# OxfordML/GPz

Measured on AMD Instinct MI355X. Metric: objective+gradient evals/sec, higher is better.
Workload: dtype f64

## Files before the change

gpz_amd/csrc/gpz_ctx.h:

```cpp
#pragma once
#include <hip/hip_runtime.h>
#include <math.h>
#include <stdarg.h>
#include <stdio.h>
#include <stdlib.h>
#include <string.h>
#include <algorithm>
#include <atomic>
#include <mutex>
#include <string>
#include <type_traits>
#include <vector>
#include "../../include/gpz_hip.h"
#include "gpz_dev.h"
#include "gpz_kernels.h"
#include <map>

#define HIPCHK(x)                                                                                   \
    do {                                                                                            \
        hipError_t e_ = (x);                                                                        \
        if (e_ != hipSuccess) return gpz_fail(GPZ_ERR_HIP, "%s:%d %s: %s", __FILE__, __LINE__, #x, hipGetErrorString(e_)); \
    } while (0)

inline int method_id_of(const char *m) {
// ... 129 lines not shown
    }
    hipEvent_t get() {
        if (pool_used == pool.size()) {
            hipEvent_t e;
            (void)hipEventCreate(&e);
            pool.push_back(e);
        }
        return pool[pool_used++];
    }
};

struct gpz_ctx {
    gpz_desc desc;
    gpz_options opt = gpz_options_load();
    int mid = 0, kind = 0, d = 0, de = 0, m = 0, mp = 0, mq = 0, k = 1, hetero = 0, g_dim = 0;
    long p = 0;
    int device = 0;
    hipStream_t st = nullptr;
    Arena ar;
    RowSet tr, va;
    double *theta_d = nullptr;
    GpzParams pr{};
    double *Phi = nullptr, *T = nullptr, *dL = nullptr;
    double *lnbeta = nullptr, *wbeta = nullptr, *phiw = nullptr;
    double *lnbeta_v = nullptr, *phiw_v = nullptr;
    double *slab = nullptr;
    size_t slab_count = 0;
    int nsplit = 1, rows_per_split = 16;
    int nsplit_d = 1, rows_per_split_d = 16;
    int nsplit_l = 1, rows_per_split_l = 16;
    double *comm1 = nullptr;
    size_t comm1_count = 0;
    double *comm2 = nullptr;
    size_t comm2_count = 0;
    int nm = 0;
    double *A = nullptr, *Lm = nullptr, *Wm = nullptr, *Tmp = nullptr, *Sinv = nullptr, *Bext = nullptr;
    float *Bext32 = nullptr;
    char *oz_A = nullptr, *oz_B = nullptr;
    double *oz_cs = nullptr;
    double *w = nullptr, *dwda = nullptr, *dgi = nullptr, *logdet = nullptr;
    int *info = nullptr;
    double *colslab = nullptr, *scal_slab = nullptr;
    int nwg_rows = 1;
    double *mom_slab = nullptr;
    int nchunk = 1, rows_per_chunk = 1;
    int tile_rows = 0, ntiles = 1, tile_nchunk = 1, tile_rpc = 1;
    double *tile_rstats = nullptr;
    double *partial = nullptr, *rstats = nullptr, *dGfull = nullptr, *spart = nullptr;
    double *nupart = nullptr, *rowscal = nullptr, *frec = nullptr;
    bool syrk_small = false;
    bool small_tail_dp = false;
    bool small_tail = false;
    int st_nwg = 0, st_nf = 0;
    double *st_slab = nullptr;
    bool fused = true;
    double *phipart = nullptr;
    int phipart_groups = 0;
    long phipart_rows = 0;
    int nslots = 0;
    double *out_d = nullptr;
    double *out_h = nullptr, *theta_h = nullptr;
    gpz_allreduce_fn ar_fn = nullptr;
    void *ar_user = nullptr;
    void *priv = nullptr;
    void (*priv_free)(void *) = nullptr;
    int timing = 0;
    bool time_rest = false;
    struct GraphSeg {
        hipGraphExec_t exec = nullptr;
        int stage = -1;
        bool count_call = false;
        double *hook_buf = nullptr;
        size_t hook_count = 0;
    };
    struct GraphSet { std::vector<GraphSeg> segs; int state = 0; };
    GraphSet gset[2];
    GraphSet *cap = nullptr;
    int cap_stage = -1;
    bool cap_stage_first = false, cap_failed = false;
    hipStream_t graph_st = nullptr;
    bool capturing = false;
    StageTimer tm;
    bool phi_valid = false;
    bool has_psi = false, has_missing = false;
    int pinv_mode = 0;
    double *g_dev_out = nullptr;
    double pinv_last[4] = {0, 0, 0, 0};
    bool gen = false;
    bool psi_fast = false;
    bool psi_miss = false;
    bool psi32 = false;
    int psi_kind_in = 0;
    bool need_psi3 = true;
    bool psi32_agreed = false;
    int ngroups = 0, nrec = 0;
    std::vector<std::vector<unsigned char>> pats;
    bool pats_fixed = false;
    unsigned char *pat_d = nullptr;
    double *prep_ws = nullptr;
    double *Sig = nullptr, *iSig = nullptr, *lnS = nullptr, *Phi_v = nullptr, *gen_slab = nullptr, *psi32_raw = nullptr;
    double *gc_minv = nullptr;
    double *gcq_A = nullptr, *gcq_B = nullptr;
    double *RcP = nullptr, *gen_tslab = nullptr, *gen_frec = nullptr, *fin_part = nullptr;
    double *gen_ws = nullptr;
    int gen_tnch = 1;
    int *mom_chunktab = nullptr, *mom_segtab = nullptr;
// ... 66 lines not shown
```

gpz_amd/csrc/gpz_ctx.hip:

```cpp
#include "gpz_ctx.h"

namespace gpzi {
static int upload_rowset(gpz_ctx *c, RowSet &rs, int64_t n_tot, const double *X, const double *Y, const double *omega,
                         const uint8_t *mask, bool need_xr, const double *Psi = nullptr) {
    const int d = c->d, de = c->de, k = c->k;
    std::vector<int64_t> idx;
    idx.reserve((size_t)n_tot);
    for (int64_t i = 0; i < n_tot; ++i)
        if (!mask || mask[i]) idx.push_back(i);
    if (c->gen) {
        std::vector<int> hg0(idx.size());
        for (size_t r = 0; r < idx.size(); ++r) {
            std::vector<unsigned char> pt(d);
            for (int c_ = 0; c_ < d; ++c_) { const double xv = X[(size_t)c_ * n_tot + idx[r]]; pt[c_] = (xv != xv) ? 0 : 1; }
            int g = -1;
            for (size_t q = 0; q < c->pats.size(); ++q)
                if (c->pats[q] == pt) { g = (int)q; break; }
            if (g < 0) {
                if (c->pats_fixed) return gpz_fail(GPZ_ERR_ARG, "row %lld has a NaN pattern that is not in the given pattern table", (long long)idx[r]);
                c->pats.push_back(pt);
                g = (int)c->pats.size() - 1;
            }
            hg0[r] = g;
        }
// ... 464 lines not shown
        int target = rows_at(1024) >= 16384 ? 1024 : rows_at(512) >= 4096 ? 512 : 256;
        if (c->opt.syrk_wgs > 0) target = c->opt.syrk_wgs;
        const int noff = npairs - nt, max_ns = np_k / 64 > 0 ? (int)(np_k / 64) : 1;
        int s1 = 1, s2 = 1;
        double best = 1e300;
        for (int a = 1; a <= max_ns && a <= target && noff * a + nt <= (target > npairs ? target : npairs); ++a) {
            int b = noff ? (target - noff * a) / nt : a;
            if (b > max_ns) b = max_ns;
            if (b > a) b = a;
            if (b < 1) b = 1;
            const double cost = 1.0 / a > 0.6 / b ? 1.0 / a : 0.6 / b;
            if (cost < best) { best = cost; s1 = a; s2 = b; }
        }
        if (c->opt.syrk_s1 > 0) s1 = c->opt.syrk_s1;
        if (c->opt.syrk_s2 > 0) s2 = c->opt.syrk_s2;
        c->rows_per_split = rup((int)((np_k + s1 - 1) / s1), 16);
        c->nsplit = (int)((np_k + c->rows_per_split - 1) / c->rows_per_split);
        c->rows_per_split_d = rup((int)((np_k + s2 - 1) / s2), 16);
        c->nsplit_d = (int)((np_k + c->rows_per_split_d - 1) / c->rows_per_split_d);
        size_t need = (size_t)(c->nsplit > c->nsplit_d ? c->nsplit : c->nsplit_d) * mp * mp;
        c->syrk_small = syrk_small_fits(mp) && !c->psi32 && !c->opt.syrk_small_off;
        if (c->syrk_small) {
            const size_t ns = syrk_small_slab_count((int)np_k, mp);
            if (ns > need) need = ns;
        }
        size_t need_l = (size_t)c->nsplit_l * c->mq * c->mq;
        c->slab_count = need > need_l ? need : need_l;
        if ((rc = c->ar.alloc(&c->slab, c->slab_count))) return bail(rc);
    }
    {
        size_t prow = npt < 1024 * 1024 ? npt : 0;
        if (c->va.n_pad && (size_t)c->va.n_pad < 1024 * 1024 && (size_t)c->va.n_pad > prow) prow = (size_t)c->va.n_pad;
        if (prow) {
            c->phipart_groups = 16;
            c->phipart_rows = (long)prow;
            if ((rc = c->ar.alloc(&c->phipart, (size_t)c->phipart_groups * 2 * k * prow))) return bail(rc);
        }
    }
    c->comm1_count = k * mp * mp + gpz_ns(c->k);
    if ((rc = c->ar.alloc(&c->comm1, c->comm1_count))) return bail(rc);
    c->comm2_count = m * c->nm + k * 2 * mp + k * 4 + gpz_ns(c->k);
    if ((rc = c->ar.alloc(&c->comm2, c->comm2_count))) return bail(rc);
    c->nwg_rows = c->tr.n < 2048 ? (c->tr.n > 0 ? c->tr.n : 1) : 2048;
    if (!c->fused) {
        if ((rc = c->ar.alloc(&c->colslab, (size_t)c->nwg_rows * 2 * mp))) return bail(rc);
        if ((rc = c->ar.alloc(&c->scal_slab, (size_t)c->nwg_rows * 4))) return bail(rc);
    } else {
        c->nslots = gpz_gemm_wave_cols() * ((c->mp + 127) / 128);
        if ((rc = c->ar.alloc(&c->nupart, (size_t)c->nslots * npt))) return bail(rc);
        if ((rc = c->ar.alloc(&c->rowscal, (size_t)4 * np))) return bail(rc);
        if ((rc = c->ar.alloc(&c->frec, (size_t)m * (c->nm + 2)))) return bail(rc);
    }
    {
        const int ncg = (c->m + 255) / 256;
        const int nc_env = c->opt.mom_nc;
        int nc = nc_env > 0 ? nc_env / ncg : (768 / ncg > 512 ? 768 / ncg : (2048 / ncg < 512 ? 2048 / ncg : 512));
        if (nc_env <= 0 && c->kind == GPZ_KIND_COV) {
            long rounds = ((long)c->tr.n * ncg + 1024 * 1000 - 1) / (1024 * 1000);
            if (rounds < 1) rounds = 1;
            if (rounds > 4) rounds = 4;
            nc = (int)(512 * rounds / ncg);
            if (nc < 1) nc = 1;
        }
        if (nc_env <= 0 && c->kind == GPZ_KIND_DIAG && c->m < 256) nc = nc * 256 / ((c->m + 63) / 64 * 64);
        const int max_nc = c->tr.n / 32 > 0 ? c->tr.n / 32 : 1;
        if (nc > max_nc) nc = max_nc;
        if (nc < 1) nc = 1;
        if (c->gen) nc = 1;
        c->rows_per_chunk = (c->tr.n + nc - 1) / nc;
        if (c->rows_per_chunk < 1) c->rows_per_chunk = 1;
        c->nchunk = c->tr.n > 0 ? (c->tr.n + c->rows_per_chunk - 1) / c->rows_per_chunk : 1;
        if (c->tile_rows) {
            int nct = nc;
            if (nct > c->tile_rows / 32) nct = c->tile_rows / 32 > 0 ? c->tile_rows / 32 : 1;
            c->tile_rpc = (c->tile_rows + nct - 1) / nct;
            c->tile_nchunk = (c->tile_rows + c->tile_rpc - 1) / c->tile_rpc;
            c->nchunk = c->ntiles * c->tile_nchunk;
        }
        if ((rc = c->ar.alloc(&c->mom_slab, (size_t)c->nchunk * m * (c->nm + 2)))) return bail(rc);
    }
    if ((rc = c->ar.alloc(&c->partial, (size_t)GPZ_ROWSCAL_MAX_NWG * gpz_ns(c->k)))) return bail(rc);
    static_assert(GPZ_ROWSCAL_MAX_NWG >= GPZ_SMALL_NWG, "partial record buffer");
    if ((rc = c->ar.alloc(&c->rstats, (size_t)gpz_ns(c->k)))) return bail(rc);
    if ((rc = c->ar.alloc(&c->spart, (size_t)(c->k > 8 ? c->k : 8)))) return bail(rc);
    if ((rc = c->ar.alloc(&c->dGfull, c->kind == GPZ_KIND_COV ? m * c->d * c->d : m * c->d))) return bail(rc);
    if ((rc = c->ar.alloc(&c->out_d, (size_t)c->p + 10))) return bail(rc);
    if (hipHostMalloc((void **)&c->out_h, ((size_t)c->p + 10) * sizeof(double)) != hipSuccess ||
        hipHostMalloc((void **)&c->theta_h, (size_t)c->p * sizeof(double)) != hipSuccess)
        return bail(gpz_fail(GPZ_ERR_ALLOC, "hipHostMalloc failed"));
    *out = c;
    return GPZ_OK;
}
namespace gpzi {

}
extern "C" void gpz_ctx_destroy(gpz_ctx *c) {
    if (!c) return;
    (void)hipSetDevice(c->device);
    (void)hipStreamSynchronize(c->st);
    if (c->priv && c->priv_free) c->priv_free(c->priv);
    c->ar.release();
    if (c->out_h) (void)hipHostFree(c->out_h);
    if (c->theta_h) (void)hipHostFree(c->theta_h);
    for (auto &gs : c->gset)
        for (auto &s : gs.segs)
            if (s.exec) (void)hipGraphExecDestroy(s.exec);
    if (c->graph_st) (void)hipStreamDestroy(c->graph_st);
    for (hipEvent_t e : c->tm.pool) (void)hipEventDestroy(e);
    delete c;
}
namespace gpzi {

}
bool gpz_ctx_allreduce_is(const gpz_ctx *c, int (*fn)(void *, void *, size_t, void *), void **user) {
    if (user) *user = c->ar_user;
    return c->ar_fn == fn;
}
int gpz_ctx_device(const gpz_ctx *c) { return c->device; }
void gpz_ctx_attach_private(gpz_ctx *c, void *priv, void (*free_fn)(void *)) {
    if (c->priv && c->priv_free) c->priv_free(c->priv);
    c->priv = priv;
    c->priv_free = free_fn;
}
namespace gpzi {

}
extern "C" int gpz_ctx_set_allreduce(gpz_ctx *c, gpz_allreduce_fn fn, void *user) {
    if (!c) return gpz_fail(GPZ_ERR_ARG, "null context");
    c->ar_fn = fn;
    c->ar_user = user;
    return GPZ_OK;
}
// ... 37 lines not shown
    c->timing = enable < 0 ? 0 : enable > 2 ? 2 : enable;
    c->time_rest = enable >= 3;
    return GPZ_OK;
}
namespace gpzi {
}
extern "C" int gpz_ctx_reset_timings(gpz_ctx *c) {
    if (!c) return gpz_fail(GPZ_ERR_ARG, "null context");
    for (auto &v : c->tm.ms) v = 0.0;
    for (auto &v : c->tm.calls) v = 0;
    return GPZ_OK;
}
namespace gpzi {
}
extern "C" int gpz_ctx_timings(gpz_ctx *c, const char **names, double *ms, int64_t *calls, int cap) {
    if (!c) return gpz_fail(GPZ_ERR_ARG, "null context");
    const int n = (int)c->tm.names.size();
    for (int i = 0; i < n && i < cap; ++i) {
        if (names) names[i] = c->tm.names[i];
        if (ms) ms[i] = c->tm.ms[i];
        if (calls) calls[i] = c->tm.calls[i];
    }
    return n;
}
namespace gpzi {

}
extern "C" int gpz_ctx_route(const gpz_ctx *c, char *buf, int cap) {
    if (!c || !buf || cap <= 0) return gpz_fail(GPZ_ERR_ARG, "gpz_ctx_route: null argument");
    const bool f32req = c->desc.dtype == GPZ_F32;
    const char *phi, *why = "";
    if (!c->gen) phi = c->d > 20 ? "tuned diagonal / covariance kernels, runtime-d form (k_wide)" : "tuned kernels (k_phi, k_rows)";
    else if (!c->has_psi) phi = "covariance kinds with missing dimensions: tuned kernels per NaN pattern";
    else if (c->psi32) phi = (c->tr.psi_diag && psi32m_available(c->d))
                                 ? "fp32 pair kernels: k_psi32_phi + k_psi32m_moments (4x4 MFMA tiles)" : "fp32 pair kernels (k_psi32)";
    else if (c->psi_fast) phi = c->d <= 10 ? "fp64 pair kernels in registers (k_psi)"
                                : cpsi4_available(c->d) ? "fp64 pair kernels on 4x4 f64 MFMA tiles (k_cpsi4)" : "fp64 pair kernels on MFMA tiles (k_cpsi4w / k_cpsi)";
    else phi = "fp64 pair kernels, workspace form (k_gen)";
    if (f32req && !c->psi32)
        why = !c->gen || !c->has_psi ? " [dtype f32 requested: no input noise on a covariance kind, nothing runs in fp32]"
              : c->d > 20            ? " [dtype f32 requested: d > 20 has no fp32 pair kernel, fp64 route]"
                                     : " [dtype f32 requested: rows with missing dimensions, fp64 route]";
    const int gstate = c->gset[c->timing == 2 ? 1 : 0].state;
    const size_t nseg = c->gset[c->timing == 2 ? 1 : 0].segs.size();
    char gsb[96];
    if (gstate == 2 && nseg > 1) snprintf(gsb, sizeof gsb, "replayed (%zu segments%s)", nseg, c->desc.world > 1 ? ", all-reduce between them" : "");
    else snprintf(gsb, sizeof gsb, "%s", gstate == 2 ? "replayed" : gstate == -1 ? "disabled (recording failed)" : c->opt.no_graph ? "disabled (GPZ_NO_GRAPH)"
                                         : c->timing == 1 ? "off (stage timing on)" : "eager (not recorded yet)");
    const char *gs = gsb;
    const bool f32mm = c->psi32 && !c->opt.f32_contractions_off;
    char rows[96];
    if (c->tile_rows) snprintf(rows, sizeof rows, "; rows: streamed, %d tiles of %d (PHI built twice per evaluation)", c->ntiles, c->tile_rows);
    else rows[0] = 0;
    return snprintf(buf, (size_t)cap, "pair/PHI kernels: %s%s; contractions: %s MFMA%s%s; evaluation graph: %s%s", phi, why,
                    f32mm ? "fp32-operand (fp64 master sums)" : "fp64",
                    c->syrk_small ? ", PHI' W PHI with the whole triangle in one workgroup (k_syrk_small)" : "",
                    c->small_tail ? ", T-GEMM + row scalars + moments in one kernel (k_small_tail: T stays in registers)" :
                    c->small_tail_dp ? ", T-GEMM + row scalars + dPHI in one kernel (k_small_tail; moment sums with input noise by k_moments_diag)" : "", gs, rows);
}
namespace gpzi {

}
```

gpz_amd/csrc/gpz_eval.hip:

```cpp
#include "gpz_ctx.h"

namespace gpzi {
static GenRows gen_rows(const RowSet &rs) {
    GenRows r{};
    r.Xr = rs.Xr; r.gid = rs.gid; r.Psi3 = rs.Psi3; r.rows_by_group = rs.rows_by_group; r.n = rs.n; r.n_pad = rs.n_pad;
    return r;
}

static void psi32_chunks(const gpz_ctx *c, int *nch, int *rpc) {
    int r = (c->tr.n + c->gen_nchunk - 1) / c->gen_nchunk;
    r = rup(r > 0 ? r : 1, 64);
    *rpc = r;
    *nch = c->tr.n > 0 ? (c->tr.n + r - 1) / r : 1;
}

static int allreduce(gpz_ctx *c, double *buf, size_t count) {
    if (c->desc.world <= 1) return 0;
    if (!c->ar_fn) return gpz_fail(GPZ_ERR_COMM, "world=%d but no all-reduce hook set (gpz_ctx_set_allreduce)", c->desc.world);
    if (c->capturing) {
        if (graph_cut(c)) return gpz_fail(GPZ_ERR_HIP, "evaluation graph: cut at an exchange point failed");
        c->cap->segs.back().hook_buf = buf;
        c->cap->segs.back().hook_count = count;
        return 0;
    }
// ... 261 lines not shown
        if (c->pinv_mode == 0) launch_cond_flag(c->st, S, c->mp, c->pr.alpha + (size_t)o * m, c->Sinv, mq, m, c->Tmp, c->info);
    }
}

static int stage_b_pinv(gpz_ctx *c, int o) {
    const int mq = c->mq, m = c->m;
    const double *S = c->comm1 + (size_t)o * c->mp * c->mp;
    Stage s(c, "pinv_svd");
    double *sbuf = c->Tmp, *out3 = c->Tmp + mq + 8;
    unsigned long long *word = (unsigned long long *)(c->Tmp + mq);
    const int sweeps = run_jacobi_pinv(c->st, S, c->mp, c->pr.alpha + (size_t)o * m, m, c->A, c->Wm, mq, sbuf, word, c->Sinv,
                                       mq, c->logdet + o, out3);
    if (sweeps < 0) return gpz_fail(GPZ_ERR_HIP, "pseudo-inverse (Jacobi SVD) failed: %s", hipGetErrorString(hipGetLastError()));
    double h3[3] = {0, 0, 0};
    HIPCHK(hipMemcpyAsync(h3, out3, sizeof h3, hipMemcpyDeviceToHost, c->st));
    HIPCHK(hipStreamSynchronize(c->st));
    c->pinv_last[0] = 1.0;
    c->pinv_last[1] = (o == 0) ? h3[1] : fmin(c->pinv_last[1], h3[1]);
    c->pinv_last[2] = h3[2];
    c->pinv_last[3] = (double)sweeps;
    launch_post_inverse(c->st, c->Sinv, mq, S, c->mp, c->pr.alpha + (size_t)o * m, m, c->mp, o, c->Bext,
                        c->w + (size_t)o * m, c->dwda + (size_t)o * m, c->dgi + (size_t)o * m, c->info, c->logdet);
    return 0;
}

int eval_tail(gpz_ctx *c, bool pinv) {
    const size_t mp = c->mp, m = c->m, k = c->k;
    double *mom = c->comm2;
    double *cols = mom + m * c->nm;
    double *scal = cols + k * 2 * mp;
    double *vsums = scal + k * 4;
    const bool fused = c->fused;
    for (int o = 0; o < c->k; ++o) {
        if (pinv) { if (int e = stage_b_pinv(c, o)) return e; }
        else stage_b(c, o);
        if (c->tile_rows) {
            const size_t oo = (size_t)o * c->tr.n_pad;
            for (int t = 0; t < c->ntiles; ++t) {
                const RowTile rt = row_tile(c, t);
                const long r0 = rt.r0;
                { Stage s(c, "phi_build"); if (int e = phi_tile(c, rt)) return e; }
                {
                    Stage s(c, "tgemm");
                    launch_tgemm(c->st, c->Phi, c->mp, c->Bext, c->mp, c->T, rt.rows_pad, c->mp, c->nupart, c->phiw + oo + r0, c->m, c->m + o,
                                 c->psi32 && !c->opt.f32_contractions_off);
                }
                {
                    Stage s(c, "row_scalars");
                    launch_row_scalars(c->st, c->nupart, c->nslots, c->phiw + oo + r0, c->tr.Y + oo + r0, c->tr.om ? c->tr.om + r0 : nullptr,
                                       c->lnbeta + oo + r0, c->wbeta + oo + r0, rt.rows_pad, rt.rows, c->rowscal + 4 * r0, c->partial, (long)o * c->tr.om_ld);
                    launch_slab_sum(c->st, c->partial, row_scalars_nwg(rt.rows), GPZ_NS, c->tile_rstats + (size_t)t * GPZ_NS);
                }
                Stage s(c, "moments");
                FusedMomentArgs a{};
                a.Phi = c->Phi; a.T = c->T; a.ld = c->mp; a.Xr = c->tr.Xr + r0 * c->de; a.rowscal = c->rowscal + 4 * r0; a.n = rt.rows;
                a.m = c->m; a.d = c->de; a.kind = c->kind; a.P = c->pr.P; a.w = c->w + (size_t)o * m;
                a.v = c->hetero ? c->pr.v + (size_t)o * m : nullptr;
                a.rows_per_chunk = c->tile_rpc; a.nchunk = (rt.rows + c->tile_rpc - 1) / c->tile_rpc;
                a.slab = c->mom_slab + (size_t)t * c->tile_nchunk * m * (c->nm + 2); a.nm = c->nm;
                a.Psir = c->tr.Psir ? c->tr.Psir + r0 * c->de : nullptr; a.Mr = c->tr.Mr ? c->tr.Mr + r0 * c->de : nullptr; a.G2 = c->pr.G2;
                if (a.nchunk > 0 && launch_moments_fused(c->st, a))
                    return gpz_fail(GPZ_ERR_UNSUPPORTED, "moment kernel not instantiated for d=%d", c->de);
            }
            Stage s(c, "moments");
            launch_slab_sum(c->st, c->tile_rstats, c->ntiles, GPZ_NS, c->rstats);
            HIPCHK(hipMemcpyAsync(scal + (size_t)o * 4, c->rstats, 4 * sizeof(double), hipMemcpyDeviceToDevice, c->st));
            const RowTile last = row_tile(c, c->ntiles - 1);
            const int nch = (c->ntiles - 1) * c->tile_nchunk + (last.rows + c->tile_rpc - 1) / c->tile_rpc;
            launch_slab_sum(c->st, c->mom_slab, nch, m * (c->nm + 2), c->frec);
            launch_split_fused(c->st, c->frec, c->m, c->nm, c->mp, mom, cols + (size_t)o * 2 * mp, o > 0 ? 1 : 0);
            continue;
        }
        if (c->small_tail_dp) {
            {
                Stage s(c, "tail_small");
                SmallTailArgs a{};
                a.Phi = c->Phi; a.ld = c->mp; a.B = c->Bext; a.ldb = c->mp;
                a.n = c->tr.n; a.n_pad = c->tr.n_pad; a.m = c->m; a.mp = c->mp; a.d = c->de; a.kind = c->kind; a.mcol = c->m;
                a.Xs = c->tr.Xs; a.xs_ld = c->tr.xs_ld; a.missing = 0;
                a.y = c->tr.Y; a.omega = c->tr.om; a.omega1 = c->tr.om; a.lnbeta = c->lnbeta; a.wbeta = c->wbeta;
                a.w = c->w; a.v = c->hetero ? c->pr.v : c->w; a.vscale = c->hetero ? 1.0 : 0.0;
                a.phiw = c->phiw; a.slab = c->st_slab; a.partial = c->partial; a.nf = 0; a.stagger = c->opt.small_stagger;
                a.dphi = c->T; a.ldd = c->mp;
                launch_small_tail(c->st, a, c->st_nwg);
                launch_small_finish(c->st, c->st_slab, c->partial, c->st_nwg, c->m, c->de, c->kind, 0, 0, c->pr.P, c->tr.xmu, c->nm, c->mp, mom,
                                    cols, scal, 0, 1);
            }
            Stage s(c, "moments");
            MomentArgs ma{};
            ma.dPhi = c->T; ma.ld = c->mp; ma.Xr = c->tr.Xr; ma.n = c->tr.n; ma.n_pad = c->tr.n_pad; ma.m = c->m; ma.d = c->de;
            ma.kind = c->kind; ma.P = c->pr.P; ma.nchunk = c->nchunk; ma.rows_per_chunk = c->rows_per_chunk; ma.slab = c->mom_slab;
            ma.nm = c->nm; ma.Psir = c->tr.Psir; ma.Mr = c->tr.Mr; ma.G2 = c->pr.G2;
            if (launch_moments(c->st, ma)) return gpz_fail(GPZ_ERR_UNSUPPORTED, "moment kernel not instantiated for d=%d", c->de);
            launch_slab_sum(c->st, c->mom_slab, c->nchunk, m * c->nm, mom);
            continue;
        }
        if (c->small_tail) {
            Stage s(c, "tail_small");
            const size_t oo = (size_t)o * c->tr.n_pad;
            SmallTailArgs a{};
            a.Phi = c->Phi; a.ld = c->mp; a.B = c->Bext; a.ldb = c->mp;
            a.n = c->tr.n; a.n_pad = c->tr.n_pad; a.m = c->m; a.mp = c->mp; a.d = c->de; a.kind = c->kind; a.mcol = c->m + o;
            a.Xs = c->tr.Xs; a.xs_ld = c->tr.xs_ld; a.missing = c->has_missing ? 1 : 0;
            a.y = c->tr.Y + oo; a.omega = c->tr.om ? c->tr.om + (size_t)o * c->tr.om_ld : nullptr; a.omega1 = c->tr.om;
            a.lnbeta = c->lnbeta + oo; a.wbeta = c->wbeta + oo;
            a.w = c->w + (size_t)o * m; a.v = c->hetero ? c->pr.v + (size_t)o * m : a.w; a.vscale = c->hetero ? 1.0 : 0.0;
            a.phiw = c->phiw + oo; a.slab = c->st_slab; a.partial = c->partial; a.nf = c->st_nf; a.stagger = c->opt.small_stagger;
            launch_small_tail(c->st, a, c->st_nwg);
            launch_small_finish(c->st, c->st_slab, c->partial, c->st_nwg, c->m, c->de, c->kind, c->st_nf, c->has_missing ? 1 : 0, c->pr.P,
                                c->tr.xmu, c->nm, c->mp, mom, cols + (size_t)o * 2 * mp, scal + (size_t)o * 4, o > 0 ? 1 : 0);
            continue;
        }
        {
            Stage s(c, "tgemm");
            const bool f32mm = c->psi32 && !c->opt.f32_contractions_off;
#ifdef GPZ_DEV_SWITCHES
            if (c->oz_A && !f32mm) {
                if (o == 0) launch_oz_slice_a(c->st, c->Phi, c->mp, (long)c->tr.n_pad, c->m, c->mp, c->oz_A);
                launch_oz_slice_b(c->st, c->Bext, c->mp, c->mp, c->mp, c->oz_cs, c->oz_B);
                launch_oz_tgemm(c->st, c->oz_A, c->oz_B, c->oz_cs, c->Phi, c->mp, c->T, c->mp, (long)c->tr.n_pad, c->mp,
                                fused ? c->nupart : nullptr, fused ? c->phiw + (size_t)o * c->tr.n_pad : c->phiw, c->m, c->m + o);
// ... 19 lines not shown
            if (c->gen && !c->has_psi) {
                if (int e = moments_by_pattern(c, true, mom)) return e;
                continue;
            }
            if (c->gen && c->psi32) {
                int nch, rpc;
                psi32_chunks(c, &nch, &rpc);
                if (c->tr.psi_diag && psi32m_available(c->d))
                    launch_psi32m_moments(c->st, c->Phi, c->T, c->mp, c->rowscal, c->w, c->hetero ? c->pr.v : nullptr, c->tr.Xr,
                                          c->de, c->d, c->tr.PsiT, (long)c->tr.n_pad, c->tr.n, c->m, c->pr.P, c->pr.Rc, nch, rpc,
                                          c->gen_slab);
                else
                    launch_psi32_moments(c->st, c->Phi, c->T, c->mp, c->rowscal, c->w, c->hetero ? c->pr.v : nullptr, c->tr.Xr,
                                         c->de, c->d, c->tr.PsiT, (long)c->tr.n_pad, c->tr.psi_diag, c->tr.n, c->m, c->pr.P, c->Sig,
                                         c->pr.Rc, nch, rpc, c->gen_slab, c->nrec);
                launch_slab_sum(c->st, c->gen_slab, nch, m * psi32_raw_len(c->d), c->psi32_raw);
                launch_psi32_records(c->st, c->psi32_raw, c->d, c->tr.psi_diag, c->m, mom, c->nrec);
                continue;
            }
            if (c->gen && c->psi_fast) {
                int nch = c->gen_nchunk;
                if (nch > c->tr.n) nch = c->tr.n;
                if (nch < 1) nch = 1;
                const int rpc = (c->tr.n + nch - 1) / nch > 0 ? (c->tr.n + nch - 1) / nch : 1;
                nch = (c->tr.n + rpc - 1) / rpc;
                if (nch < 1) nch = 1;
                if (c->psi_miss) {
                    launch_psi_moments(c->st, c->Phi, c->T, c->mp, c->rowscal, c->w, c->hetero ? c->pr.v : nullptr,
                                       gen_rows(c->tr), c->m, c->d, c->de, c->pr.P, c->Sig, c->mom_nchunk, 0, c->gen_slab,
                                       c->nrec, c->pat_d, c->mom_chunktab, c->gc_minv);
                    launch_slab_sum_seg(c->st, c->gen_slab, c->mom_segtab, c->ngroups, m * c->nrec, mom);
                    continue;
                }
                launch_psi_moments(c->st, c->Phi, c->T, c->mp, c->rowscal, c->w, c->hetero ? c->pr.v : nullptr,
                                   gen_rows(c->tr), c->m, c->d, c->de, c->pr.P, c->Sig, nch, rpc, c->gen_slab, c->nrec,
                                   nullptr, nullptr, c->gc_minv);
                launch_slab_sum(c->st, c->gen_slab, nch, m * c->nrec, mom);
                continue;
            }
            if (c->gen) {
                const GenRows gr = gen_rows(c->tr);
                for (int g = 0; g < c->ngroups; ++g) {
                    const int rb = c->tr.group_begin[g], nr = c->tr.group_begin[g + 1] - rb;
                    double *recs_g = mom + (size_t)g * m * c->nrec;
                    if (nr <= 0) { launch_zero(c->st, recs_g, m * c->nrec); continue; }
                    int nch = c->gen_nchunk;
                    if (nch > nr) nch = nr;
                    const int rpc = (nr + nch - 1) / nch;
                    nch = (nr + rpc - 1) / rpc;
                    launch_gen_moments(c->st, c->Phi, c->T, c->mp, c->rowscal, c->w, c->hetero ? c->pr.v : nullptr, gr, g, rb,
                                       nr, c->pat_d, c->m, c->d, c->de, c->pr.P, c->Sig, nch, rpc, c->gen_slab, c->nrec, c->gen_ws);
                    launch_slab_sum(c->st, c->gen_slab, nch, m * c->nrec, recs_g);
                }
                continue;
            }
            FusedMomentArgs a{};
            a.Phi = c->Phi; a.T = c->T; a.ld = c->mp; a.Xr = c->tr.Xr; a.rowscal = c->rowscal; a.n = c->tr.n; a.m = c->m;
            a.d = c->de; a.kind = c->kind; a.P = c->pr.P; a.w = c->w + (size_t)o * m;
            a.v = c->hetero ? c->pr.v + (size_t)o * m : nullptr;
            a.nchunk = c->nchunk; a.rows_per_chunk = c->rows_per_chunk; a.slab = c->mom_slab; a.nm = c->nm;
            a.Psir = c->tr.Psir; a.Mr = c->tr.Mr; a.G2 = c->pr.G2;
            if (launch_moments_fused(c->st, a))
                return gpz_fail(GPZ_ERR_UNSUPPORTED, "moment kernel not instantiated for d=%d", c->de);
            launch_slab_sum(c->st, c->mom_slab, c->nchunk, m * (c->nm + 2), c->frec);
            launch_split_fused(c->st, c->frec, c->m, c->nm, c->mp, mom, cols + (size_t)o * 2 * mp, o > 0 ? 1 : 0);
            continue;
        }
        {
            Stage s(c, "row_epilogue");
            RowArgs a{};
            a.Phi = c->Phi; a.T = c->T; a.ld = c->mp; a.n = c->tr.n; a.m = c->m; a.mp = c->mp; a.k = c->k; a.out = o;
            a.y = c->tr.Y; a.omega = c->tr.om; a.om_ld = c->tr.om_ld; a.lnbeta = c->lnbeta; a.wbeta = c->wbeta; a.ldx = c->tr.n_pad;
            a.w = c->w + (size_t)o * m; a.v = c->hetero ? c->pr.v + (size_t)o * m : nullptr;
            a.dL = c->dL; a.colslab = c->colslab; a.scal = c->scal_slab; a.nwg = c->nwg_rows;
            launch_row_epilogue(c->st, a);
            launch_colslab_reduce(c->st, c->colslab, c->scal_slab, c->nwg_rows, c->mp, cols + (size_t)o * 2 * mp,
                                  scal + (size_t)o * 4);
        }
    }
    if (!fused) {
        {
            Stage s(c, "mul_phi");
            launch_mul_phi(c->st, c->dL, c->Phi, c->T, (size_t)c->tr.n_pad * mp);
        }
        Stage s(c, "moments");
        if (c->gen && !c->has_psi) {
            if (int e = moments_by_pattern(c, false, mom)) return e;
        } else if (c->gen && c->psi32) {
            int nch, rpc;
            psi32_chunks(c, &nch, &rpc);
            if (c->tr.psi_diag && psi32m_available(c->d))
                launch_psi32m_moments(c->st, c->Phi, c->T, c->mp, nullptr, nullptr, nullptr, c->tr.Xr, c->de, c->d, c->tr.PsiT,
                                      (long)c->tr.n_pad, c->tr.n, c->m, c->pr.P, c->pr.Rc, nch, rpc, c->gen_slab);
            else
                launch_psi32_moments(c->st, c->Phi, c->T, c->mp, nullptr, nullptr, nullptr, c->tr.Xr, c->de, c->d, c->tr.PsiT,
                                     (long)c->tr.n_pad, c->tr.psi_diag, c->tr.n, c->m, c->pr.P, c->Sig, c->pr.Rc, nch, rpc,
                                     c->gen_slab, c->nrec);
            launch_slab_sum(c->st, c->gen_slab, nch, m * psi32_raw_len(c->d), c->psi32_raw);
            launch_psi32_records(c->st, c->psi32_raw, c->d, c->tr.psi_diag, c->m, mom, c->nrec);
        } else if (c->gen && c->psi_fast) {
            int nch = c->gen_nchunk;
            if (nch > c->tr.n) nch = c->tr.n;
            if (nch < 1) nch = 1;
            const int rpc = (c->tr.n + nch - 1) / nch > 0 ? (c->tr.n + nch - 1) / nch : 1;
            nch = (c->tr.n + rpc - 1) / rpc;
            if (nch < 1) nch = 1;
// ... 193 lines not shown
```

gpz_amd/csrc/gpz_kernels.h:

```cpp
#pragma once
#include <hip/hip_runtime.h>
#include <stdint.h>
#include "gpz_options.h"

struct gpz_ctx;
int gpz_fail(int code, const char *fmt, ...);
void gpz_ctx_attach_private(gpz_ctx *c, void *priv, void (*free_fn)(void *));
bool gpz_ctx_allreduce_is(const gpz_ctx *c, int (*fn)(void *, void *, size_t, void *), void **user);
int gpz_ctx_device(const gpz_ctx *c);

struct GpzParams {
    double *P;
    double *G;
    double *G2;
    double *Rc;
    double *lnAlpha;
    double *alpha;
    double *b;
    double *v;
    double *lnTau;
    double *tau;
};

void launch_unpack(hipStream_t st, const double *theta, int method_id, int m, int d, int de, int k, int hetero,
// ... 126 lines not shown

void launch_fill_bext(hipStream_t st, const double *Sinv, int ldsi, const double *w, int m, int mp, int out,
                      double *Bext, double *dgi);

struct RowArgs {
    const double *Phi; double *T; int ld;
    int n, m, mp, k, out;
    const double *y, *omega, *lnbeta, *wbeta; long ldx;
    long om_ld;
    const double *w, *v;
    double *dL;
    double *colslab;
    double *scal;
    int nwg;
};
void launch_row_epilogue(hipStream_t st, const RowArgs &a);
void launch_colslab_reduce(hipStream_t st, const double *colslab, const double *scal, int nwg, int mp, double *out_cols,
                           double *out_scal);
void launch_mul_phi(hipStream_t st, const double *dL, const double *Phi, double *T, size_t count);

struct MomentArgs {
    const double *dPhi; int ld;
    const double *Xr;
    int n, n_pad, m, d, kind;
    const double *P;
    int nchunk, rows_per_chunk;
    double *slab;
    int nm;
    const double *Psir, *Mr, *G2;
    const int *chunktab;
};
int launch_moments(hipStream_t st, const MomentArgs &a);

#define GPZ_ROWSCAL_MAX_NWG 1024
inline int row_scalars_nwg(int n) {
    const int w = (n + 511) / 512;
    return w < 128 ? 128 : (w > GPZ_ROWSCAL_MAX_NWG ? GPZ_ROWSCAL_MAX_NWG : w);
}
void launch_row_scalars(hipStream_t st, const double *nupart, int nslots, const double *phiw, const double *y,
                        const double *omega, const double *lnbeta, const double *wbeta, long n_pad, int n,
                        double *rowscal, double *partial, long om_off = 0);
struct FusedMomentArgs {
    const double *Phi, *T; int ld;
    const double *Xr, *rowscal;
    int n, m, d, kind;
    const double *P, *w, *v;
    int nchunk, rows_per_chunk;
    double *slab;
    int nm;
    const double *Psir, *Mr, *G2;
    const int *chunktab;
};
int launch_moments_fused(hipStream_t st, const FusedMomentArgs &a);
int launch_moments_wide(hipStream_t st, const MomentArgs &a);
int launch_moments_fused_wide(hipStream_t st, const FusedMomentArgs &a);
void launch_split_fused(hipStream_t st, const double *rec, int m, int nm, int mp, double *mom, double *cols,
                        int accumulate = 0 );
void launch_slab_sum(hipStream_t st, const double *slab, int nslab, size_t count, double *out);
void launch_slab_sum_seg(hipStream_t st, const double *slab, const int *seg, int nseg, size_t count, double *out);

struct FinishArgs {
    int method_id, kind, m, d, k, hetero, g_dim;
    GpzParams pr;
    const double *mom; int nm;
    const double *cols;
    const double *scal;
    const double *w, *dwda, *dgi;
    const double *logdet;
    const double *sums1;
    const double *vsums;
    const int *info;
    double *out;
    double *dGfull;
    int p;
    int nmp;
    int de;
    int psi;
    int gen;
};
void launch_finish(hipStream_t st, const FinishArgs &a);

#define GPZ_NS 12
__host__ __device__ inline int gpz_ns(int k) { return GPZ_NS + (k > 8 ? k - 8 : 0); }
__host__ __device__ inline int gpz_ns_idx(int base, int o) { return o < 8 ? base + o : GPZ_NS + (o - 8); }
#define GPZ_SMALL_NWG 128
void launch_row_stats(hipStream_t st, const double *phiw, const double *y, const double *omega, long om_ld, const double *lnbeta,
                      long ldx, int n, int k, double *partial);
void launch_sums1(hipStream_t st, const double *omega, long om_ld, const double *lnbeta, long ldx, int n, int k, double *partial);
void launch_solve_partial(hipStream_t st, GpzParams pr, const double *w, const double *logdet, const double *sums1,
                          const double *rstats, int m, int k, double *out);
size_t nan_groups_work_bytes(long n, int d);
int launch_nan_groups(hipStream_t st, const double *X, long n, int d, void *work ,
                      int *n_groups, int *group_id);

struct GenRows {
    const double *Xr;
    const int *gid;
    const double *Psi3;
    const int *rows_by_group;
    int n, n_pad;
};
size_t gen_ws_per_thread(int d);
int gen_rt_threads(int d);
void launch_gen_prep(hipStream_t st, const double *G, int m, int d, int de, double *Sig, double *iSig,
                     const unsigned char *pat, int ngroups, double *lnS, double *ws = nullptr);
void launch_gen_pattern_params(hipStream_t st, const double *Sig, const double *P, const unsigned char *pat, int G, int m,
// ... 167 lines not shown
```

gpz_amd/csrc/gpz_options.h:

```cpp
#pragma once

struct gpz_options {
    bool no_graph = false;
    bool graph_debug = false;
    long row_tile = 0;
    long cache_cap_mb = -1;
    bool psi32_mfma = false;
    long predict_min_rows_per_block = 4096;
    bool f32_contractions_off = false;
    bool gc_minv_off = false;
    bool gc_dense_phi_off = false;
    bool tgemm_no_split = false;
    bool phi_diag_no_split = false;
    bool pmc_scratch = false;
    bool pmc_prep_scratch = false;
    bool pmc_no_model_cache = false;
    bool round_phi32 = false;
    bool cpsi_off = false;
    bool cpsi4_off = false;
    bool tgemm_int8 = false;
    int syrk_wgs = 0, syrk_s1 = 0, syrk_s2 = 0;
    int mom_nc = 0;
    int small_stagger = 0;
    bool chol_rowinv_off = false;
    bool syrk_small_off = false;
    bool small_tail_off = false;
    int debug_fail_cut = 0;
};

gpz_options gpz_options_load();

const gpz_options &gpz_opts();
struct gpz_opts_scope {
    const gpz_options *prev;
    explicit gpz_opts_scope(const gpz_options *o);
    ~gpz_opts_scope();
    gpz_opts_scope(const gpz_opts_scope &) = delete;
    gpz_opts_scope &operator=(const gpz_opts_scope &) = delete;
};
```

gpz_amd/csrc/gpz_options.hip:

```cpp
#include <stdlib.h>
#include "gpz_options.h"

static const char *env(const char *name) { return getenv(name); }
static bool env_set(const char *name) { return env(name) != nullptr; }
static long env_long(const char *name, long dflt) {
    const char *e = env(name);
    return e ? atol(e) : dflt;
}

gpz_options gpz_options_load() {
    gpz_options o;
    o.no_graph = env_set("GPZ_NO_GRAPH");
    o.graph_debug = env_set("GPZ_GRAPH_DEBUG");
    o.row_tile = env_long("GPZ_ROW_TILE", 0);
    o.cache_cap_mb = env_long("GPZ_CACHE_CAP_MB", -1);
    {
        const char *e = env("GPZ_PSI32_MFMA");
        o.psi32_mfma = e && e[0] == '1';
    }
    o.predict_min_rows_per_block = env_long("GPZ_PREDICT_MIN_ROWS_PER_BLOCK", 4096);
    if (o.predict_min_rows_per_block < 1) o.predict_min_rows_per_block = 1;
#ifdef GPZ_DEV_SWITCHES
    o.f32_contractions_off = env_set("GPZ_F32_CONTRACTIONS_OFF");
    o.gc_minv_off = env_set("GPZ_GC_MINV_OFF");
    o.gc_dense_phi_off = env_set("GPZ_GC_DENSE_PHI_OFF");
    o.tgemm_no_split = env_set("GPZ_TGEMM_NO_SPLIT");
    o.phi_diag_no_split = env_set("GPZ_PHI_DIAG_NO_SPLIT");
    o.pmc_scratch = env_set("GPZ_PMC_SCRATCH");
    o.pmc_prep_scratch = env_set("GPZ_PMC_PREP_SCRATCH");
    o.pmc_no_model_cache = env_set("GPZ_PMC_NO_MODEL_CACHE");
    o.round_phi32 = env_set("GPZ_EXPERIMENT_ROUND_PHI32");
    o.cpsi_off = env_set("GPZ_CPSI_OFF");
    o.cpsi4_off = env_set("GPZ_CPSI4_OFF");
    o.tgemm_int8 = env_set("GPZ_TGEMM_INT8");
    o.syrk_wgs = (int)env_long("GPZ_SYRK_WGS", 0);
    o.syrk_s1 = (int)env_long("GPZ_SYRK_S1", 0);
    o.syrk_s2 = (int)env_long("GPZ_SYRK_S2", 0);
    o.mom_nc = (int)env_long("GPZ_MOM_NC", 0);
    o.debug_fail_cut = (int)env_long("GPZ_DEBUG_FAIL_CUT", 0);
    o.small_tail_off = env_set("GPZ_SMALL_TAIL_OFF");
    o.syrk_small_off = env_set("GPZ_SYRK_SMALL_OFF");
    o.chol_rowinv_off = env_set("GPZ_CHOL_ROWINV_OFF");
    o.small_stagger = (int)env_long("GPZ_SMALL_STAGGER", 0);
#endif
    return o;
}

static thread_local const gpz_options *t_opts = nullptr;
const gpz_options &gpz_opts() {
    if (t_opts) return *t_opts;
    static const gpz_options process = gpz_options_load();
    return process;
}
gpz_opts_scope::gpz_opts_scope(const gpz_options *o) : prev(t_opts) { t_opts = o; }
gpz_opts_scope::~gpz_opts_scope() { t_opts = prev; }
```

Baseline: 18.37.

## Add LDS-ring moments kernel with async global-to-LDS staging for COV d=8/10

Adds a new moments kernel for the covariance case with d of 8 or 10. It streams PHI, T, the inputs and the row scalars into a per-wave 4-slot LDS ring using global_load_lds and manual vmcnt waits. It accumulates raw (uncentered) feature moments with f64 MFMA, and a finish kernel reduces the chunk records and applies the centering about P per column. This replaces the fused moments plus slab-sum plus split path and is meant to hide memory latency and shrink record width, at the cost of a narrow-applicability specialised path that depends on hand-tuned waitcnt counts.

Measured after the change: 18.68 (median of 6 runs). 1.7% higher.

```diff
diff --git a/gpz_amd/csrc/gpz_ctx.h b/gpz_amd/csrc/gpz_ctx.h
--- a/gpz_amd/csrc/gpz_ctx.h
+++ b/gpz_amd/csrc/gpz_ctx.h
@@ -205,6 +205,8 @@
     bool small_tail_dp = false;
     bool small_tail = false;
     int st_nwg = 0, st_nf = 0;
+    bool mom_ring = false;
+    int mom_nv = 0;
     double *st_slab = nullptr;
     bool fused = true;
     double *phipart = nullptr;
diff --git a/gpz_amd/csrc/gpz_ctx.hip b/gpz_amd/csrc/gpz_ctx.hip
--- a/gpz_amd/csrc/gpz_ctx.hip
+++ b/gpz_amd/csrc/gpz_ctx.hip
@@ -540,7 +540,9 @@
         if ((rc = c->ar.alloc(&c->frec, (size_t)m * (c->nm + 2)))) return bail(rc);
     }
     {
-        const int ncg = (c->m + 255) / 256;
+        c->mom_ring = c->fused && !c->gen && !c->has_psi && !c->has_missing && !c->small_tail && !c->small_tail_dp && c->tr.Xs &&
+                      c->tr.xs_ld == c->de + 2 && moments_ring_fits(c->kind, c->de, c->mp) && !c->opt.moments_ring_off;
+        const int ncg = c->mom_ring ? (c->m + moments_ring_cols() - 1) / moments_ring_cols() : (c->m + 255) / 256;
         const int nc_env = c->opt.mom_nc;
         int nc = nc_env > 0 ? nc_env / ncg : (768 / ncg > 512 ? 768 / ncg : (2048 / ncg < 512 ? 2048 / ncg : 512));
         if (nc_env <= 0 && c->kind == GPZ_KIND_COV) {
@@ -565,7 +567,8 @@
             c->tile_nchunk = (c->tile_rows + c->tile_rpc - 1) / c->tile_rpc;
             c->nchunk = c->ntiles * c->tile_nchunk;
         }
-        if ((rc = c->ar.alloc(&c->mom_slab, (size_t)c->nchunk * m * (c->nm + 2)))) return bail(rc);
+        c->mom_nv = c->mom_ring ? moments_ring_features(c->de) + 2 : c->nm + 2;
+        if ((rc = c->ar.alloc(&c->mom_slab, (size_t)c->nchunk * m * c->mom_nv))) return bail(rc);
     }
     if ((rc = c->ar.alloc(&c->partial, (size_t)GPZ_ROWSCAL_MAX_NWG * gpz_ns(c->k)))) return bail(rc);
     static_assert(GPZ_ROWSCAL_MAX_NWG >= GPZ_SMALL_NWG, "partial record buffer");
@@ -709,12 +712,13 @@
     char rows[96];
     if (c->tile_rows) snprintf(rows, sizeof rows, "; rows: streamed, %d tiles of %d (PHI built twice per evaluation)", c->ntiles, c->tile_rows);
     else rows[0] = 0;
-    return snprintf(buf, (size_t)cap, "pair/PHI kernels: %s%s; contractions: %s MFMA%s%s; evaluation graph: %s%s", phi, why,
+    return snprintf(buf, (size_t)cap, "pair/PHI kernels: %s%s; contractions: %s MFMA%s%s; evaluation graph: %s%s%s", phi, why,
                     f32mm ? "fp32-operand (fp64 master sums)" : "fp64",
                     c->syrk_small ? ", PHI' W PHI with the whole triangle in one workgroup (k_syrk_small)" : "",
                     c->small_tail ? ", T-GEMM + row scalars + moments in one kernel (k_small_tail: T stays in registers)" :
-                    c->small_tail_dp ? ", T-GEMM + row scalars + dPHI in one kernel (k_small_tail; moment sums with input noise by k_moments_diag)" : "", gs, rows);
-}
-namespace gpzi {
-
-}
+                    c->small_tail_dp ? ", T-GEMM + row scalars + dPHI in one kernel (k_small_tail; moment sums with input noise by k_moments_diag)" : "", gs, rows,
+                    c->mom_ring ? "; moments: k_moments_ring (PHI, T through an LDS ring)" : "");
+}
+namespace gpzi {
+
+}
diff --git a/gpz_amd/csrc/gpz_eval.hip b/gpz_amd/csrc/gpz_eval.hip
--- a/gpz_amd/csrc/gpz_eval.hip
+++ b/gpz_amd/csrc/gpz_eval.hip
@@ -337,6 +337,15 @@
                     launch_slab_sum(c->st, c->partial, row_scalars_nwg(rt.rows), GPZ_NS, c->tile_rstats + (size_t)t * GPZ_NS);
                 }
                 Stage s(c, "moments");
+                if (c->mom_ring) {
+                    RingMomentArgs ra{};
+                    ra.Phi = c->Phi; ra.T = c->T; ra.ld = c->mp; ra.Xs = c->tr.Xs + r0 * c->tr.xs_ld; ra.rowscal = c->rowscal + 4 * r0;
+                    ra.n = rt.rows; ra.m = c->m; ra.d = c->de; ra.w = c->w + (size_t)o * m; ra.v = c->hetero ? c->pr.v + (size_t)o * m : nullptr;
+                    ra.rows_per_chunk = c->tile_rpc; ra.nchunk = (rt.rows + c->tile_rpc - 1) / c->tile_rpc;
+                    ra.slab = c->mom_slab + (size_t)t * c->tile_nchunk * m * c->mom_nv;
+                    if (launch_moments_ring(c->st, ra)) return gpz_fail(GPZ_ERR_HIP, "k_moments_ring launch failed (d=%d)", c->de);
+                    continue;
+                }
                 FusedMomentArgs a{};
                 a.Phi = c->Phi; a.T = c->T; a.ld = c->mp; a.Xr = c->tr.Xr + r0 * c->de; a.rowscal = c->rowscal + 4 * r0; a.n = rt.rows;
                 a.m = c->m; a.d = c->de; a.kind = c->kind; a.P = c->pr.P; a.w = c->w + (size_t)o * m;
@@ -352,6 +361,10 @@
             HIPCHK(hipMemcpyAsync(scal + (size_t)o * 4, c->rstats, 4 * sizeof(double), hipMemcpyDeviceToDevice, c->st));
             const RowTile last = row_tile(c, c->ntiles - 1);
             const int nch = (c->ntiles - 1) * c->tile_nchunk + (last.rows + c->tile_rpc - 1) / c->tile_rpc;
+            if (c->mom_ring) {
+                launch_ring_finish(c->st, c->mom_slab, nch, c->m, c->de, c->pr.P, c->tr.xmu, c->nm, c->mp, mom, cols + (size_t)o * 2 * mp, o > 0 ? 1 : 0);
+                continue;
+            }
             launch_slab_sum(c->st, c->mom_slab, nch, m * (c->nm + 2), c->frec);
             launch_split_fused(c->st, c->frec, c->m, c->nm, c->mp, mom, cols + (size_t)o * 2 * mp, o > 0 ? 1 : 0);
             continue;
@@ -477,6 +490,15 @@
                                        nr, c->pat_d, c->m, c->d, c->de, c->pr.P, c->Sig, nch, rpc, c->gen_slab, c->nrec, c->gen_ws);
                     launch_slab_sum(c->st, c->gen_slab, nch, m * c->nrec, recs_g);
                 }
+                continue;
+            }
+            if (c->mom_ring) {
+                RingMomentArgs ra{};
+                ra.Phi = c->Phi; ra.T = c->T; ra.ld = c->mp; ra.Xs = c->tr.Xs; ra.rowscal = c->rowscal; ra.n = c->tr.n; ra.m = c->m; ra.d = c->de;
+                ra.w = c->w + (size_t)o * m; ra.v = c->hetero ? c->pr.v + (size_t)o * m : nullptr;
+                ra.nchunk = c->nchunk; ra.rows_per_chunk = c->rows_per_chunk; ra.slab = c->mom_slab;
+                if (launch_moments_ring(c->st, ra)) return gpz_fail(GPZ_ERR_HIP, "k_moments_ring launch failed (d=%d)", c->de);
+                launch_ring_finish(c->st, c->mom_slab, c->nchunk, c->m, c->de, c->pr.P, c->tr.xmu, c->nm, c->mp, mom, cols + (size_t)o * 2 * mp, o > 0 ? 1 : 0);
                 continue;
             }
             FusedMomentArgs a{};
diff --git a/gpz_amd/csrc/gpz_kernels.h b/gpz_amd/csrc/gpz_kernels.h
--- a/gpz_amd/csrc/gpz_kernels.h
+++ b/gpz_amd/csrc/gpz_kernels.h
@@ -202,6 +202,21 @@
     const int *chunktab;
 };
 int launch_moments_fused(hipStream_t st, const FusedMomentArgs &a);
+struct RingMomentArgs {
+    const double *Phi, *T; int ld;
+    const double *Xs;
+    const double *rowscal;
+    int n, m, d;
+    const double *w, *v;
+    int nchunk, rows_per_chunk;
+    double *slab;
+};
+bool moments_ring_fits(int kind, int de, int mp);
+int moments_ring_cols();
+int moments_ring_features(int de);
+int launch_moments_ring(hipStream_t st, const RingMomentArgs &a);
+void launch_ring_finish(hipStream_t st, const double *slab, int nrec, int m, int d, const double *P, const double *xmu, int nm, int mp,
+                        double *mom, double *cols, int accumulate);
 int launch_moments_wide(hipStream_t st, const MomentArgs &a);
 int launch_moments_fused_wide(hipStream_t st, const FusedMomentArgs &a);
 void launch_split_fused(hipStream_t st, const double *rec, int m, int nm, int mp, double *mom, double *cols,
diff --git a/gpz_amd/csrc/gpz_options.h b/gpz_amd/csrc/gpz_options.h
--- a/gpz_amd/csrc/gpz_options.h
+++ b/gpz_amd/csrc/gpz_options.h
@@ -25,6 +25,7 @@
     bool chol_rowinv_off = false;
     bool syrk_small_off = false;
     bool small_tail_off = false;
+    bool moments_ring_off = false;
     int debug_fail_cut = 0;
 };
 
diff --git a/gpz_amd/csrc/gpz_options.hip b/gpz_amd/csrc/gpz_options.hip
--- a/gpz_amd/csrc/gpz_options.hip
+++ b/gpz_amd/csrc/gpz_options.hip
@@ -42,6 +42,7 @@
     o.syrk_small_off = env_set("GPZ_SYRK_SMALL_OFF");
     o.chol_rowinv_off = env_set("GPZ_CHOL_ROWINV_OFF");
     o.small_stagger = (int)env_long("GPZ_SMALL_STAGGER", 0);
+    o.moments_ring_off = env_set("GPZ_MOMENTS_RING_OFF");
 #endif
     return o;
 }
diff --git a/gpz_amd/csrc/k_moments_ring.hip b/gpz_amd/csrc/k_moments_ring.hip
--- /dev/null
+++ b/gpz_amd/csrc/k_moments_ring.hip
@@ -0,0 +1,246 @@
+#include "gpz_dev.h"
+#include "gpz_kernels.h"
+
+#define RG_ROWS 8
+#define RG_SLOTS 4
+#define RG_JB 2
+#define RG_COLS 32
+#define RG_SLOT_DOUBLES 640
+#define RG_SIDE 512
+#define RG_SIDE_RS 96
+#define RG_GROUP_REQ 5
+#define RG_LDS_BYTES 81920
+#define RG_GLDS(g, l) __builtin_amdgcn_global_load_lds((const __attribute__((address_space(1))) void *)(g), (__attribute__((address_space(3))) void *)(l), 16, 0, 0)
+static_assert(RG_LDS_BYTES == 4 * RG_SLOTS * RG_SLOT_DOUBLES * 8 && RG_COLS == 16 * RG_JB && RG_SIDE == 2 * RG_ROWS * RG_COLS, "ring size");
+
+template <int D>
+__global__ __launch_bounds__(256, 2) void k_moments_ring(RingMomentArgs a) {
+    constexpr int NF = 1 + D + D * (D + 1) / 2, XL = D + 2;
+    constexpr int NFB = NF >= 64 ? NF / 16 : (NF + 15) / 16;
+    constexpr int NL = NF > 16 * NFB ? NF - 16 * NFB : 0;
+    static_assert(RG_ROWS * XL <= RG_SIDE_RS, "side block");
+    extern __shared__ double rg_smem[];
+    const int tid = threadIdx.x, lane = tid & 63, wave = __builtin_amdgcn_readfirstlane(tid >> 6), li = lane & 15, lk = lane >> 4;
+    const int ncg = (a.m + 4 * RG_COLS - 1) / (4 * RG_COLS);
+    const int cg = blockIdx.x % ncg, chunk = blockIdx.x / ncg;
+    const int j0 = cg * (4 * RG_COLS) + wave * RG_COLS;
+    if (j0 >= a.m) return;
+    double *const ring = rg_smem + wave * (RG_SLOTS * RG_SLOT_DOUBLES);
+    const int r_begin = chunk * a.rows_per_chunk;
+    const int r_end = min(a.n, r_begin + a.rows_per_chunk);
+    const int ng = (r_end - r_begin + RG_ROWS - 1) / RG_ROWS;
+    double wj[RG_JB], vj[RG_JB];
+#pragma unroll
+    for (int cb = 0; cb < RG_JB; ++cb) {
+        const int j = min(j0 + 16 * cb + li, a.m - 1);
+        wj[cb] = a.w[j];
+        vj[cb] = a.v ? a.v[j] : 0.0;
+    }
+    int fia[NFB], fib[NFB];
+#pragma unroll
+    for (int fb = 0; fb < NFB; ++fb) {
+        const int f = 16 * fb + li;
+        int ia = 0, ib = 0;
+        if (f >= NF) ia = ib = XL - 1;
+        else if (f >= 1) {
+            if (f <= D) ia = f;
+            else {
+                int e2 = f - 1 - D, aa = 0;
+                while (e2 >= D - aa) { e2 -= D - aa; ++aa; }
+                ia = aa + 1; ib = aa + e2 + 1;
+            }
+        }
+        fia[fb] = ia; fib[fb] = ib;
+    }
+    int lia[NL > 0 ? NL : 1], lib[NL > 0 ? NL : 1];
+#pragma unroll
+    for (int t = 0; t < NL; ++t) {
+        int e2 = 16 * NFB + t - 1 - D, aa = 0;
+        while (e2 >= D - aa) { e2 -= D - aa; ++aa; }
+        lia[t] = aa + 1; lib[t] = aa + e2 + 1;
+    }
+    d4_t acc[RG_JB][NFB];
+    double ev[RG_JB][NL + 2];
+#pragma unroll
+    for (int cb = 0; cb < RG_JB; ++cb) {
+#pragma unroll
+        for (int fb = 0; fb < NFB; ++fb) acc[cb][fb] = d4_t{0.0, 0.0, 0.0, 0.0};
+#pragma unroll
+        for (int t = 0; t < NL + 2; ++t) ev[cb][t] = 0.0;
+    }
+    const unsigned colj = (unsigned)min(j0 + 2 * (lane & 15), a.ld - 2);
+    const unsigned voff = (unsigned)(lane >> 4) * (unsigned)a.ld + colj;
+    const bool is_rs = lane >= 48;
+    const unsigned soff = is_rs ? 2u * (unsigned)(lane - 48) : min(2u * (unsigned)lane, (unsigned)(RG_ROWS * XL - 2));
+    const double *const sbase = is_rs ? a.rowscal : a.Xs;
+    const unsigned srow = is_rs ? 4u : (unsigned)XL;
+    const long last = (long)r_end - 1;
+    auto stage_half = [&](int g, int slot, int h) {
+        const long rg = (long)r_begin + (long)g * RG_ROWS + 4 * h;
+        double *const l0 = ring + slot * RG_SLOT_DOUBLES + 4 * h * RG_COLS;
+        if (rg + 4 <= (long)r_end) {
+            const size_t ro = (size_t)rg * (size_t)a.ld;
+            RG_GLDS(a.Phi + ro + voff, l0);
+            RG_GLDS(a.T + ro + voff, l0 + RG_ROWS * RG_COLS);
+        } else {
+            long row = rg + (lane >> 4);
+            row = row < last ? row : last;
+            const size_t ro = (size_t)row * (size_t)a.ld + colj;
+            RG_GLDS(a.Phi + ro, l0);
+            RG_GLDS(a.T + ro, l0 + RG_ROWS * RG_COLS);
+        }
+    };
+    auto stage_side = [&](int g, int slot) {
+        const long rg = (long)r_begin + (long)g * RG_ROWS;
+        double *const l0 = ring + slot * RG_SLOT_DOUBLES + RG_SIDE;
+        long e = rg * (long)srow + (long)soff;
+        const long elast = (long)r_end * (long)srow - 2;
+        e = e < elast ? e : elast;
+        RG_GLDS(sbase + e, l0);
+    };
+    auto kstep = [&](const double *s0, int kk, int rows_left) {
+        const int rr = 4 * kk + lk;
+        const bool valid = rr < rows_left;
+        const double *xr = s0 + RG_SIDE + rr * XL;
+        const double *rs = s0 + RG_SIDE + RG_SIDE_RS + rr * 4;
+        const double r0 = rs[0], r1 = rs[1], r2 = rs[2];
+        const double ob = valid ? r0 : 0.0, cc = valid ? r1 : 0.0, db = valid ? r2 : 0.0;
+        double fr[NFB], fl[NL > 0 ? NL : 1];
+#pragma unroll
+        for (int fb = 0; fb < NFB; ++fb) fr[fb] = xr[fia[fb]] * xr[fib[fb]];
+#pragma unroll
+        for (int t = 0; t < NL; ++t) fl[t] = xr[lia[t]] * xr[lib[t]];
+        const double *pp = s0 + rr * RG_COLS + li;
+        double phn = pp[0], ttn = pp[RG_ROWS * RG_COLS];
+        __builtin_amdgcn_sched_barrier(0);
+#pragma unroll
+        for (int cb = 0; cb < RG_JB; ++cb) {
+            const double ph = phn, tt = ttn;
+            if (cb + 1 < RG_JB) { phn = pp[16 * (cb + 1)]; ttn = pp[RG_ROWS * RG_COLS + 16 * (cb + 1)]; }
+            const double dp = fma(-ob, tt, fma(db, vj[cb], -cc * wj[cb])) * ph;
+#pragma unroll
+            for (int fb = 0; fb < NFB; ++fb) acc[cb][fb] = MFMA_F64(dp, fr[fb], acc[cb][fb]);
+#pragma unroll
+            for (int t = 0; t < NL; ++t) ev[cb][t] = fma(dp, fl[t], ev[cb][t]);
+            ev[cb][NL] = fma(ph, cc, ev[cb][NL]);
+            ev[cb][NL + 1] = fma(ph, db, ev[cb][NL + 1]);
+            __builtin_amdgcn_sched_barrier(0);
+        }
+    };
+    for (int g = 0; g < RG_SLOTS; ++g)
+        if (g < ng) { stage_half(g, g, 0); stage_half(g, g, 1); stage_side(g, g); }
+    for (int g = 0; g < ng; ++g) {
+        const int ahead = ng - 1 - g;
+        if (ahead >= 3) asm volatile("s_waitcnt vmcnt(15)" ::: "memory");
+        else if (ahead == 2) asm volatile("s_waitcnt vmcnt(10)" ::: "memory");
+        else if (ahead == 1) asm volatile("s_waitcnt vmcnt(5)" ::: "memory");
+        else asm volatile("s_waitcnt vmcnt(0)" ::: "memory");
+        const int slot = g % RG_SLOTS;
+        const double *s0 = ring + slot * RG_SLOT_DOUBLES;
+        const int rows_left = r_end - r_begin - g * RG_ROWS;
+        const bool more = g + RG_SLOTS < ng;
+        kstep(s0, 0, rows_left);
+        asm volatile("s_waitcnt lgkmcnt(0)" ::: "memory");
+        if (more) stage_half(g + RG_SLOTS, slot, 0);
+        kstep(s0, 1, rows_left);
+        asm volatile("s_waitcnt lgkmcnt(0)" ::: "memory");
+        if (more) { stage_half(g + RG_SLOTS, slot, 1); stage_side(g + RG_SLOTS, slot); }
+    }
+    double *rec = a.slab + (size_t)chunk * a.m * (NF + 2);
+#pragma unroll
+    for (int cb = 0; cb < RG_JB; ++cb) {
+#pragma unroll
+        for (int r = 0; r < 4; ++r) {
+            const int j = j0 + 16 * cb + lk + 4 * r;
+            if (j < a.m) {
+                double *o = rec + (size_t)j * (NF + 2);
+#pragma unroll
+                for (int fb = 0; fb < NFB; ++fb)
+                    if (16 * fb + li < NF) o[16 * fb + li] = acc[cb][fb][r];
+            }
+        }
+        const int j = j0 + 16 * cb + li;
+#pragma unroll
+        for (int t = 0; t < NL + 2; ++t) {
+            double s = ev[cb][t];
+            s += __shfl_xor(s, 16, 64);
+            s += __shfl_xor(s, 32, 64);
+            if (lk == 0 && j < a.m) rec[(size_t)j * (NF + 2) + (NF - NL) + t] = s;
+        }
+    }
+}
+
+__global__ __launch_bounds__(1024) void k_ring_finish(const double *__restrict__ slab, int nrec, int m, int d, int nf, const double *__restrict__ P,
+                                                      const double *__restrict__ xmu, int nm, int mp, double *__restrict__ mom,
+                                                      double *__restrict__ cols, int accumulate) {
+    __shared__ double part[32][72];
+    __shared__ double R[72];
+    const int tid = threadIdx.x, j = blockIdx.x, nv = nf + 2;
+    const int L = 1024 / nv < 32 ? 1024 / nv : 32;
+    const int f = tid % nv, sl = tid / nv;
+    if (sl < L) {
+        const double *p = slab + (size_t)j * nv + f;
+        const size_t stride = (size_t)m * nv;
+        double s0 = 0.0, s1 = 0.0, s2 = 0.0, s3 = 0.0;
+        int r = sl;
+        for (; r + 3 * L < nrec; r += 4 * L) {
+            s0 += p[(size_t)r * stride];
+            s1 += p[(size_t)(r + L) * stride];
+            s2 += p[(size_t)(r + 2 * L) * stride];
+            s3 += p[(size_t)(r + 3 * L) * stride];
+        }
+        for (; r < nrec; r += L) s0 += p[(size_t)r * stride];
+        part[sl][f] = (s0 + s1) + (s2 + s3);
+    }
+    __syncthreads();
+    if (tid < nv) {
+        double t = 0.0;
+        for (int q = 0; q < L; ++q) t += part[q][tid];
+        R[tid] = t;
+    }
+    __syncthreads();
+    const int q = tid;
+    if (q >= nm + 2) return;
+    if (q >= nm) {
+        cols[(size_t)(q - nm) * mp + j] = R[nf + (q - nm)];
+        return;
+    }
+    double val;
+    if (q < d) {
+        const double qc = P[(size_t)j * d + q] - xmu[q];
+        val = R[1 + q] - qc * R[0];
+    } else {
+        int e = q - d, aa = 0;
+        while (e >= d - aa) { e -= d - aa; ++aa; }
+        const int bb = aa + e;
+        const double qa = P[(size_t)j * d + aa] - xmu[aa], qb = P[(size_t)j * d + bb] - xmu[bb];
+        val = R[1 + q] - qa * R[1 + bb] - qb * R[1 + aa] + qa * qb * R[0];
+    }
+    mom[(size_t)j * nm + q] = accumulate ? mom[(size_t)j * nm + q] + val : val;
+}
+
+bool moments_ring_fits(int kind, int de, int mp) { return kind == GPZ_KIND_COV && (de == 8 || de == 10) && mp > 256; }
+int moments_ring_cols() { return 4 * RG_COLS; }
+int moments_ring_features(int de) { return 1 + de + de * (de + 1) / 2; }
+
+template <int D>
+static int ring_launch(hipStream_t st, const RingMomentArgs &a, dim3 g) {
+    if (hipFuncSetAttribute((const void *)k_moments_ring<D>, hipFuncAttributeMaxDynamicSharedMemorySize, RG_LDS_BYTES) != hipSuccess) return -1;
+    hipLaunchKernelGGL(k_moments_ring<D>, g, dim3(256), RG_LDS_BYTES, st, a);
+    return hipGetLastError() == hipSuccess ? 0 : -1;
+}
+
+int launch_moments_ring(hipStream_t st, const RingMomentArgs &a) {
+    if (a.nchunk <= 0) return 0;
+    dim3 g((unsigned)((a.m + 4 * RG_COLS - 1) / (4 * RG_COLS)) * (unsigned)a.nchunk);
+    switch (a.d) {
+        case 8: return ring_launch<8>(st, a, g);
+        case 10: return ring_launch<10>(st, a, g);
+        default: return -1;
+    }
+}
+
+void launch_ring_finish(hipStream_t st, const double *slab, int nrec, int m, int d, const double *P, const double *xmu, int nm, int mp,
+                        double *mom, double *cols, int accumulate) {
+    hipLaunchKernelGGL(k_ring_finish, dim3(m), dim3(1024), 0, st, slab, nrec, m, d, moments_ring_features(d), P, xmu, nm, mp, mom, cols, accumulate);
+}
```
